# Mathiasb17/Nereus

Hardware: AMD Instinct MI355X
Metric: particle-steps/sec, SESPH dam-break (higher is better)
Workload: dtype f32

## Files before the change

### include/nereus_hip.h

```cpp
#ifndef NEREUS_HIP_H
#define NEREUS_HIP_H

#include <stddef.h>
#include <stdint.h>

#ifdef __cplusplus
extern "C" {
#endif

typedef struct nrs_params_f32 {
    uint32_t gridSize[3];
    uint32_t numCells;
    float worldOrigin[3];
    float cellSize[3];
    uint32_t numBodies;
    uint32_t maxParticlesPerCell;
    float gasStiffness, viscosity, surfaceTension, restDensity, particleMass, interactionRadius, timestep,
        particleRadius;
    float gravity[3];
    float soundSpeed;
    float beta;
    float kpoly, kpoly_grad, kpress_grad, kvisc_grad, kvisc_denum, ksurf1, ksurf2, bpol;
} nrs_params_f32;

// ... 14 lines not shown

typedef struct nrs_ctx nrs_ctx;

enum { NRS_SOLVER_SESPH = 0, NRS_SOLVER_IISPH = 1, NRS_SOLVER_PCISPH = 2, NRS_SOLVER_PBF = 3, NRS_SOLVER_DFSPH = 4 };
enum { NRS_KERNELS_MONAGHAN = 0, NRS_KERNELS_MULLER = 1 };

enum {
    NRS_FLAG_REFERENCE_ORDER = 1u << 0,
    NRS_FLAG_NO_FUSION = 1u << 2,
    NRS_FLAG_NO_SHARED_LISTS = 1u << 3,
    NRS_FLAG_FULL_SORT = 1u << 4,
    NRS_FLAG_FAST_ARITH = 1u << 5,
    NRS_FLAG_IISPH_SELF_BY_SLOT = 1u << 6,
    NRS_FLAG_NO_WALL_WORKGROUPS = 1u << 7,
    NRS_FLAG_STAGED_SCAN = 1u << 8,
    NRS_FLAG_IISPH_INPLACE_P = 1u << 1,
};

enum {
    NRS_OK = 0,
    NRS_E_INVALID = -1,
    NRS_E_HIP = -2,
    NRS_E_CAPACITY = -3,
    NRS_E_STATE = -4,
    NRS_E_NODEVICE = -5,
    NRS_E_NOTREADY = -6,
};

typedef struct nrs_config {
    uint32_t struct_size;
// ... 115 lines not shown

int nrs_slab_configure(nrs_ctx *ctx, int32_t cell_lo, int32_t cell_hi, int32_t halo_cells);
int nrs_slab_pack(nrs_ctx *ctx, void *send_left, void *send_right, uint64_t capacity, uint32_t counts[6]);
int nrs_slab_unpack(nrs_ctx *ctx, const void *recv_left, const void *recv_right, uint64_t capacity);
int nrs_slab_last_counts(nrs_ctx *ctx, uint32_t counts[6]);
uint64_t nrs_num_owned(nrs_ctx *ctx);
uint64_t nrs_slab_message_bytes(uint64_t capacity, int precision);
int nrs_slab_histogram(nrs_ctx *ctx, int32_t first_cell, uint32_t ncells, uint32_t *counts);

int nrs_iisph_predict(nrs_ctx *ctx);
int nrs_iisph_iterate(nrs_ctx *ctx, double *sum_density_corr, uint64_t *count);
int nrs_iisph_finish(nrs_ctx *ctx);

int nrs_resort_stats(nrs_ctx *ctx, uint64_t *steps, uint64_t *fallbacks);

enum { NRS_STAT_MOVERS = 0, NRS_STAT_HIT_OVERFLOW = 1, NRS_STAT_HIT_MEAN = 2, NRS_STAT_HIT_MAX = 3, NRS_STAT_UNSTAGED = 4,
       NRS_STAT_DENSITY_ERROR = 5, NRS_STAT_PCISPH_DELTA = 6, NRS_STAT_PBF_EPSILON = 7, NRS_STAT_DFSPH_DENSITY_AVG = 8,
       NRS_STAT_DFSPH_DIVERGENCE_AVG = 9, NRS_STAT_DFSPH_DIVERGENCE_ITERATIONS = 10, NRS_STAT_SLAB_PARTITION = 11 };
int nrs_get_stat(nrs_ctx *ctx, int which, double *out);

enum { NRS_FIELD_DENSITY = 1, NRS_FIELD_GRADIENT = 2, NRS_FIELD_VELOCITY = 4, NRS_FIELD_COUNT = 8, NRS_FIELD_WALLS = 16 };
typedef struct nrs_lattice { double origin[3]; double spacing[3]; uint32_t dims[3]; uint32_t reserved; } nrs_lattice;
int nrs_sample_points(nrs_ctx *ctx, const void *points4, uint64_t m, uint32_t fields);
int nrs_sample_lattice(nrs_ctx *ctx, const nrs_lattice *lattice, uint32_t fields);
int nrs_sample_result(nrs_ctx *ctx, uint32_t field, void *dst, uint64_t dst_bytes, uint64_t *out_bytes);
int nrs_sample_device_ptr(nrs_ctx *ctx, uint32_t field, void **dptr, uint64_t *bytes);
int nrs_sample_release(nrs_ctx *ctx);
int nrs_sample_builds(nrs_ctx *ctx, uint64_t *builds);

enum { NRS_SURFACE_GRADIENT = 1, NRS_SURFACE_VELOCITY = 2, NRS_SURFACE_WALLS = 4 };
// ... 68 lines not shown
```

### nereus_amd/capi.py

```python
import ctypes as C
import os

import numpy as np

from .params import params_dtype

_HERE = os.path.dirname(os.path.abspath(__file__))
LIB_PATH = os.environ.get("NEREUS_HIP_LIB") or os.path.join(_HERE, "libnereus_hip.so")

SESPH, IISPH, PCISPH, PBF, DFSPH = 0, 1, 2, 3, 4
MONAGHAN, MULLER = 0, 1
FLAG_REFERENCE_ORDER = 1
FLAG_NO_FUSION = 4
FLAG_NO_SHARED_LISTS = 8
FLAG_FULL_SORT = 16
FLAG_FAST_ARITH = 32
FLAG_IISPH_SELF_BY_SLOT = 64
FLAG_NO_WALL_WORKGROUPS = 128
FLAG_STAGED_SCAN = 256
MAX_BODIES = 16
E_NOTREADY = -6
STAT_MOVERS, STAT_HIT_OVERFLOW, STAT_HIT_MEAN, STAT_HIT_MAX, STAT_UNSTAGED = 0, 1, 2, 3, 4
STAT_DENSITY_ERROR, STAT_PCISPH_DELTA, STAT_PBF_EPSILON = 5, 6, 7
STAT_DFSPH_DENSITY_AVG, STAT_DFSPH_DIVERGENCE_AVG, STAT_DFSPH_DIVERGENCE_ITERATIONS = 8, 9, 10
STAT_SLAB_PARTITION = 11
FIELD_DENSITY, FIELD_GRADIENT, FIELD_VELOCITY, FIELD_COUNT, FIELD_WALLS = 1, 2, 4, 8, 16
SURFACE_GRADIENT, SURFACE_VELOCITY, SURFACE_WALLS = 1, 2, 4
MESH_VERTICES, MESH_TRIANGLES, MESH_GRADIENT, MESH_VELOCITY = 1, 2, 4, 8
ANISO_CENTER, ANISO_G, ANISO_COUNT, ANISO_INDEX = 1, 2, 4, 8
DIFFUSE_POS, DIFFUSE_VEL, DIFFUSE_KIND, DIFFUSE_POTENTIALS, DIFFUSE_BIRTHS, DIFFUSE_NORMALS = 0, 1, 2, 3, 4, 5
DIFFUSE_SPRAY, DIFFUSE_FOAM, DIFFUSE_BUBBLE = 0, 1, 2
MAX_EMITTERS, MAX_SINK_BOXES = 16, 16
EMITTER_RECT, EMITTER_DISC = 0, 1
SINK_DOMAIN = 1
# ... 11 lines not shown
    "cellStart": (5, "u"), "cellEnd": (6, "u"), "sortedPos": (7, "v4"), "sortedVel": (8, "v4"),
    "dens": (9, "s"), "pres": (10, "s"), "forces": (11, "v4"), "bhash": (12, "u"), "bindex": (13, "u"),
    "bCellStart": (14, "u"), "bCellEnd": (15, "u"), "bSorted": (16, "v4"),
    "densAdv": (20, "s"), "densCorr": (21, "s"), "P_l": (22, "s"), "aii": (23, "s"), "velAdv": (24, "v4"),
    "forcesAdv": (25, "v4"), "forcesP": (26, "v4"), "diiFluid": (27, "v4"), "diiBoundary": (28, "v4"),
    "sumDij": (29, "v4"), "posPred": (30, "v4"), "vorticity": (31, "v4"), "dfsphAlpha": (32, "s"), "dfsphKappaV": (33, "s"),
    "normals": (34, "v4"), "b_body": (35, "u"),
}

EXPORTS = [
    "nrs_last_error", "nrs_version", "nrs_device_count", "nrs_create", "nrs_destroy", "nrs_set_params",
    "nrs_get_params", "nrs_upload_particles", "nrs_set_num_particles", "nrs_num_particles", "nrs_set_boundaries",
    "nrs_step", "nrs_step_partial", "nrs_synchronize", "nrs_download", "nrs_get_array", "nrs_device_ptr",
    "nrs_last_iterations", "nrs_set_max_iterations", "nrs_set_profiling", "nrs_stage_ms", "nrs_max_density",
    "nrs_max_velocity", "nrs_slab_configure", "nrs_slab_pack", "nrs_slab_unpack", "nrs_num_owned",
    "nrs_slab_message_bytes", "nrs_slab_histogram", "nrs_resort_stats", "nrs_snapshot_begin", "nrs_snapshot_wait",
    "nrs_get_stat", "nrs_boundary_volumes", "nrs_eval_smoothing", "nrs_iisph_predict", "nrs_iisph_iterate", "nrs_iisph_finish",
    "nrs_slab_last_counts", "nrs_pcisph_configure", "nrs_pbf_configure", "nrs_pbf_set_tensile",
    "nrs_pbf_set_vorticity", "nrs_dfsph_configure", "nrs_set_surface_akinci",
    "nrs_set_boundary_bodies", "nrs_set_body_velocity", "nrs_set_body_pose", "nrs_get_body_pose",
    "nrs_sample_points", "nrs_sample_lattice", "nrs_sample_result", "nrs_sample_device_ptr", "nrs_sample_release",
    "nrs_sample_builds",
    "nrs_surface_extract", "nrs_surface_result", "nrs_surface_device_ptr", "nrs_surface_release",
    "nrs_aniso_build", "nrs_aniso_result", "nrs_aniso_device_ptr", "nrs_aniso_release", "nrs_surface_extract_aniso",
    "nrs_diffuse_configure", "nrs_diffuse_step", "nrs_diffuse_count", "nrs_diffuse_result", "nrs_diffuse_device_ptr",
    "nrs_diffuse_upload", "nrs_diffuse_release",
    "nrs_emitter_set", "nrs_emitter_get", "nrs_emit_block", "nrs_sinks_set", "nrs_cull", "nrs_sinks_count",
]


class NrsAnisoConfig(C.Structure):
# ... 88 lines not shown
    lib.nrs_set_surface_akinci.argtypes = [vp, C.c_double, C.c_double]
    lib.nrs_set_profiling.argtypes = [vp, C.c_uint32]
    lib.nrs_stage_ms.argtypes = [vp, i32, C.POINTER(C.c_float), C.POINTER(C.c_uint32)]
    lib.nrs_max_density.argtypes = [vp, C.POINTER(C.c_double)]
    lib.nrs_max_velocity.argtypes = [vp, C.POINTER(C.c_double)]
    lib.nrs_slab_configure.argtypes = [vp, C.c_int32, C.c_int32, C.c_int32]
    lib.nrs_slab_pack.argtypes = [vp, vp, vp, u64, C.POINTER(C.c_uint32)]
    lib.nrs_slab_unpack.argtypes = [vp, vp, vp, u64]
    lib.nrs_slab_last_counts.argtypes = [vp, C.POINTER(C.c_uint32)]
    lib.nrs_num_owned.argtypes = [vp]
    lib.nrs_num_owned.restype = u64
    lib.nrs_slab_message_bytes.argtypes = [u64, i32]
    lib.nrs_slab_message_bytes.restype = u64
    lib.nrs_slab_histogram.argtypes = [vp, C.c_int32, C.c_uint32, C.POINTER(C.c_uint32)]
    lib.nrs_resort_stats.argtypes = [vp, C.POINTER(u64), C.POINTER(u64)]
    lib.nrs_get_stat.argtypes = [vp, i32, C.POINTER(C.c_double)]
    lib.nrs_iisph_predict.argtypes = [vp]
    lib.nrs_iisph_iterate.argtypes = [vp, C.POINTER(C.c_double), C.POINTER(u64)]
    lib.nrs_iisph_finish.argtypes = [vp]
    lib.nrs_eval_smoothing.argtypes = [i32, i32, u64, vp, vp, C.c_double, C.c_double, C.c_double, vp]
    lib.nrs_boundary_volumes.argtypes = [i32, i32, vp, u64, C.c_double, vp]
    lib.nrs_snapshot_begin.argtypes = [vp, i32]
    lib.nrs_snapshot_wait.argtypes = [vp, i32, C.POINTER(vp), C.POINTER(vp), C.POINTER(u64), C.POINTER(u64)]
    lib.nrs_sample_points.argtypes = [vp, vp, u64, C.c_uint32]
    lib.nrs_sample_lattice.argtypes = [vp, C.POINTER(NrsLattice), C.c_uint32]
    lib.nrs_sample_result.argtypes = [vp, C.c_uint32, vp, u64, C.POINTER(u64)]
    lib.nrs_sample_device_ptr.argtypes = [vp, C.c_uint32, C.POINTER(vp), C.POINTER(u64)]
    lib.nrs_sample_release.argtypes = [vp]
    lib.nrs_sample_builds.argtypes = [vp, C.POINTER(u64)]
    lib.nrs_surface_extract.argtypes = [vp, C.POINTER(NrsLattice), C.c_double, C.c_uint32, C.POINTER(u64), C.POINTER(u64)]
# ... 257 lines not shown
        self._chk(rc)
        ct = C.c_double if self.real == np.float64 else C.c_float

        def view(ptr):
            if not ptr.value or not n.value:
                return np.empty((0, 4), self.real) if ptr.value or not n.value else None
            return np.ctypeslib.as_array(C.cast(ptr, C.POINTER(ct)), shape=(int(n.value), 4))

        return view(pp), (view(pv) if pv.value else None), int(step.value)

    def resort_stats(self):
        a, b = C.c_uint64(0), C.c_uint64(0)
        self._chk(self.lib.nrs_resort_stats(self.h, C.byref(a), C.byref(b)))
        return int(a.value), int(b.value)

    def iisph_predict(self):
        self._chk(self.lib.nrs_iisph_predict(self.h))

    def iisph_iterate(self):
        sm, cnt = C.c_double(0), C.c_uint64(0)
        self._chk(self.lib.nrs_iisph_iterate(self.h, C.byref(sm), C.byref(cnt)))
        return sm.value, int(cnt.value)

    def iisph_finish(self):
        self._chk(self.lib.nrs_iisph_finish(self.h))

    def get_stat(self, which):
        v = C.c_double()
        self._chk(self.lib.nrs_get_stat(self.h, int(which), C.byref(v)))
        return v.value
# ... 209 lines not shown
```

### nereus_amd/csrc/nrs_abi.hip

```cpp
#include "nrs_ctx_base.h"

#include <condition_variable>
#include <mutex>
#include <thread>

namespace nrs {

thread_local std::string g_err;

enum { KS_MONAGHAN_ = 0, KS_MULLER_ = 1 };
extern template CtxBase *make_ctx2<float, KS_MULLER_>(bool);
extern template CtxBase *make_ctx2<float, KS_MONAGHAN_>(bool);
extern template CtxBase *make_ctx2<double, KS_MULLER_>(bool);
extern template CtxBase *make_ctx2<double, KS_MONAGHAN_>(bool);

static CtxBase *make_ctx(const nrs_config &c)
{
    if (c.precision == 32) return c.kernel_set == NRS_KERNELS_MULLER ? make_ctx2<float, KS_MULLER_>(c.surface_tension != 0) : make_ctx2<float, KS_MONAGHAN_>(c.surface_tension != 0);
    return c.kernel_set == NRS_KERNELS_MULLER ? make_ctx2<double, KS_MULLER_>(c.surface_tension != 0) : make_ctx2<double, KS_MONAGHAN_>(c.surface_tension != 0);
}

}

using namespace nrs;
// ... 343 lines not shown
    ctx->wait_idle();
    ctx->settle_keep_error();
    return ctx->impl->num_owned();
}
int nrs_slab_histogram(nrs_ctx *ctx, int32_t first_cell, uint32_t ncells, uint32_t *counts)
{
    CTX_GUARD(ctx);
    return ctx->impl->slab_histogram(first_cell, ncells, counts);
}
int nrs_resort_stats(nrs_ctx *ctx, uint64_t *steps, uint64_t *fallbacks)
{
    CTX_GUARD(ctx);
    ctx->impl->resort_stats(steps, fallbacks);
    return NRS_OK;
}
int nrs_iisph_predict(nrs_ctx *ctx)
{
    CTX_GUARD(ctx);
    return ctx->impl->iisph_phase(0, nullptr, nullptr);
}
int nrs_iisph_iterate(nrs_ctx *ctx, double *sum_density_corr, uint64_t *count)
{
    CTX_GUARD(ctx);
    return ctx->impl->iisph_phase(1, sum_density_corr, count);
}
int nrs_iisph_finish(nrs_ctx *ctx)
{
    CTX_GUARD(ctx);
    return ctx->impl->iisph_phase(2, nullptr, nullptr);
}
// ... 170 lines not shown
```

### nereus_amd/csrc/nrs_ctx_base.h

```cpp
#pragma once
#include <cstring>
#include <hip/hip_runtime.h>

#include <cmath>
#include <cstdio>
#include <string>
#include <type_traits>
#include <utility>
#include <vector>

#include "nrs_error.h"

namespace nrs {

#define HIPCHK(expr)                                                                                     \
    do {                                                                                                 \
        hipError_t e_ = (expr);                                                                          \
        if (e_ != hipSuccess)                                                                            \
            return fail(NRS_E_HIP, std::string(#expr) + ": " + hipGetErrorString(e_) + " (" __FILE__ ":" + \
                                       std::to_string(__LINE__) + ")");                                  \
    } while (0)

struct DevBuf {
    void *p = nullptr;
// ... 75 lines not shown
    virtual int get_body_pose(uint32_t body, double *x, double *q) = 0;
    virtual int step(int nsteps, int stop) = 0;
    virtual int sync() = 0;
    virtual int download(void *pos4, void *vel4, void *pres) = 0;
    virtual int snapshot_begin(int withVel) = 0;
    virtual int snapshot_wait(int block, const void **pos4, const void **vel4, uint64_t *n, uint64_t *step) = 0;
    virtual int array(int which, void **dptr, uint64_t *bytes) = 0;
    virtual int stage_ms(int stage, float *ms, uint32_t *launches) = 0;
    virtual int reduce_max(int which, double *out) = 0;
    virtual int slab_configure(int lo, int hi, int halo) = 0;
    virtual int slab_pack(void *sendL, void *sendR, uint64_t cap, uint32_t *counts) = 0;
    virtual int slab_unpack(const void *recvL, const void *recvR, uint64_t cap) = 0;
    virtual uint64_t num_owned() = 0;
    virtual int slab_histogram(int lo0, uint32_t nbins, uint32_t *out) = 0;
    virtual void resort_stats(uint64_t *steps, uint64_t *fallbacks) = 0;
    virtual int get_stat(int which, double *out) = 0;
    virtual int iisph_phase(int phase, double *sum, uint64_t *count) = 0;
    virtual int pcisph_configure(double eta, uint32_t minIters, double spacing, double delta) = 0;
    virtual int pbf_configure(double eta, uint32_t minIters, double relaxation, double xsph) = 0;
    virtual int pbf_set_tensile(double k, double dq) = 0;
    virtual int pbf_set_vorticity(double epsV) = 0;
    virtual int dfsph_configure(double eta, uint32_t minIters, double etaV, uint32_t minItersV, int warm) = 0;
    virtual int set_surface_akinci(double gamma, double beta) = 0;
    virtual int settle() = 0;
    virtual int slab_last_counts(uint32_t *counts) = 0;
    virtual int set_profiling(uint32_t mask) = 0;
    virtual int sample_points(const void *points4, uint64_t m, uint32_t fields) = 0;
    virtual int sample_lattice(const nrs_lattice *lattice, uint32_t fields) = 0;
    virtual int sample_result(uint32_t field, void *dst, uint64_t dstBytes, uint64_t *outBytes) = 0;
    virtual int sample_device_ptr(uint32_t field, void **dptr, uint64_t *bytes) = 0;
// ... 36 lines not shown
```

### nereus_amd/csrc/nrs_ctx_impl.h

```cpp
#pragma once
#include "nrs_ctx_base.h"
#include "nrs_boundary_tables.h"
#include "nrs_host_grid.h"
#include "nrs_host_plan.h"
#include "nrs_host_profile.h"
#include "nrs_host_settings.h"
#include "nrs_host_slab.h"
#include "nrs_host_snapshot.h"
#include "nrs_host_solver.h"
#include "nrs_host_state.h"
#include "nrs_sort.h"
#include "nrs_wall_list.h"

#include "nrs_kernels_ref.h"
#include "nrs_kernels_tiled.h"
#include "nrs_kernels_staged.h"
#include <type_traits>
#include "nrs_kernels_iisph.h"
#include "nrs_kernels_pcisph.h"
#include "nrs_kernels_pbf.h"
#include "nrs_kernels_dfsph.h"
#include "nrs_kernels_akinci.h"
#include "nrs_kernels_bodies.h"
#include "nrs_slab_exchange.h"
// ... 22 lines not shown
        qOk = P.gridSize[0] >= 4u;
        for (int a = 0; a < 3; ++a) {
            qc.o[a] = (double)P.worldOrigin[a];
            qc.s[a] = QP_PER_CELL / (float)P.cellSize[a];
            const float r = (float)P.interactionRadius * qc.s[a];
            qOk = qOk && P.cellSize[a] > (R)0 && std::isfinite(qc.s[a]) && (r + QP_MARGIN < QP_HALF);
            hq = std::max(hq, r);
        }
        const double lim = (double)hq + (double)QP_MARGIN;
        qT = qOk ? (uint32_t)std::ceil(lim * lim) + 1u : 0u;
    }
    QuantCfg qc;
    uint32_t qT = 0;
    bool qOk = false;
    DevBuf gatherPos;
    DevBuf qpos;
    nrs_config cfg;
    uint64_t cap = 0, n = 0;
    bool midStep = false;
    DevBuf posA, posB, velA, velB, presA, presB, dens, forces;
    DevBuf inv;
    SortStage sort;
    DevBuf cellStart, cellEnd;
    uint32_t cellsAllocated = 0;
    BoundaryTables<R> bt;
    DevBuf densAdv, densCorr, P_l, P_l2, aii, velAdv, forcesAdv, forcesP, diiF, diiB, sumDij, diiSum;
    DevBuf redPartial, redOut;
    DevBuf posPred, posPred2, pciErr;
    DevBuf dfAlpha, dfKvA, dfKvB, dfErrV;
    DevBuf pbfVort, akNormals;
// ... 387 lines not shown
        splitClearedCells = clear;
        st.split_queued();
        NRSCHK(ev_end());
        return NRS_OK;
    }

    template <bool HAS_B> int sesph_tail(int stop)
    {
        const uint32_t N = (uint32_t)n;
        const dim3 g(nblocks(N)), b(BLOCK);
        GridView<R> G = grid_view();
        if (exch.on()) { G.actLo = exch.cuts().lo - 1; G.actHi = exch.cuts().hi + 1; }
        HitBuffer hb = hit_buffer();
        hb.gpos = gatherPos.p; hb.gvel = gatherPos.as<T4>() + 1; hb.svel = velB.p;
        if (plan.fast && !plan.staged) hb.fast = fastQ.as<FastPair>();
        const HitBuffer *share = plan.lists ? &hb : nullptr;
        const WallList wv = wall_view();
        const WallList *walls = plan.walls ? &wv : nullptr;
        if (plan.walls) {
            NRSCHK(ev_begin(NRS_STAGE_REORDER, true));
            NRSCHK(build_wall_list(N));
            NRSCHK(ev_end());
        }
        NRSCHK(ev_begin(NRS_STAGE_DENSITY));
        if (plan.ref) {
            hipLaunchKernelGGL((k_density_ref<R, KSET, HAS_B>), g, b, 0, stream, P, G, posB.as<T4>(), dens.as<R>(), presB.as<R>(), N);
        } else if (plan.staged) {
            if constexpr (std::is_same<R, float>::value)
                launch_density_staged<KSET, HAS_B>(stream, P, G, share, plan.fast, posB.as<T4>(), dens.as<R>(), presB.as<R>(),
                                                   plan.fast ? fastQ.as<FastPair>() : (FastPair *)nullptr, N);
// ... 25 lines not shown
                st.classified(N);
                sort.tile_counts_written();
            }
        }
        const FusedOut<R> *fused = plan.keys ? &fo : nullptr;
        T4 *out = plan.keys ? (T4 *)nullptr : forces.as<T4>();
        if (plan.ref) {
            hipLaunchKernelGGL((k_forces_ref<R, KSET, SURF, HAS_B>), g, b, 0, stream, P, G, posB.as<T4>(), velB.as<T4>(),
                               dens.as<R>(), presB.as<R>(), out, N);
        } else if (plan.fast) {
            if constexpr (std::is_same<R, float>::value && KSET == KS_MULLER)
                launch_forces_fast<SURF, HAS_B>(stream, P, G, hb, posB.as<T4>(), velB.as<T4>(), dens.as<R>(), presB.as<R>(),
                                                fastQ.as<FastPair>(), out, fused, N);
        } else {
            launch_forces_tiled<R, KSET, SURF, HAS_B>(stream, P, G, share, posB.as<T4>(), velB.as<T4>(), dens.as<R>(), presB.as<R>(), out,
                                                      fused, N, walls);
        }
        if (plan.keys) {
            if (!exch.on()) keys_ready();
            else sort.keys_written();
            fusedThisStep = true;
        }
        NRSCHK(ev_end());
        if (plan.resort) NRSCHK(queue_resort_split(N));
        if (stop == NRS_STAGE_FORCES || plan.keys) return NRS_OK;
        NRSCHK(ev_begin(NRS_STAGE_INTEGRATE));
        hipLaunchKernelGGL((k_integrate<R>), g, b, 0, stream, P, posB.as<T4>(), velB.as<T4>(), forces.as<T4>(), N);
        NRSCHK(ev_end());
        return NRS_OK;
    }

// ... 684 lines not shown
        st.arrivals_appended(ar.inplace, (uint32_t)ar.arrivals);
        if (!ar.inplace && st.fields().hashReady && compactResort && n >= RESORT_MIN_PARTICLES) {
            const uint32_t N = (uint32_t)n;
            NRSCHK(sort.scan_movers(nblocks(N), false));
            NRSCHK(sort.split(SplitFrom::PACKED, N, nullptr));
            st.split_queued_known(exch.host().totals[ST_CHANGED] + ar.start[5]);
        }
        exch.unpack_done();
        return NRS_OK;
    }

    void resort_stats(uint64_t *steps, uint64_t *fallbacks) override
    {
        if (steps) *steps = sort.stats().steps;
        if (fallbacks) *fallbacks = sort.stats().fallbacks;
    }
    StatFacts stat_facts() const
    {
        return StatFacts{cfg.solver, exch.host().packed, pbfSt.errPending != 0, !(pciSt.lastErr < 0.0), dfSt.denN, dfSt.divN, hitCounts.p != nullptr, n != 0, midStep};
    }
    int get_stat(int which, double *out) override
    {
        StatRoute r;
        NRSCHK(route_stat(which, stat_facts(), r));
        if (r.formMaxFirst) {
            NRSCHK(max_of<false>(pciErr.p, pbfSt.errPending, &pciSt.lastErr));
            pbfSt.errPending = 0;
            NRSCHK(route_stat(which, stat_facts(), r));
        }
        switch (r.kind) {
// ... 310 lines not shown
```

### nereus_amd/csrc/nrs_host_plan.h

```cpp
#pragma once
#include <cstdint>

#include "nrs_error.h"
#include "nrs_host_state.h"

namespace nrs {

struct PlanFacts {
    uint32_t flags;
    int solver;
    bool muller;
    bool fp32;
    uint64_t cap, n;
    bool qOk;
    bool pow2Grid;
    bool nearBitsValid;
    bool walls;
    bool slabOn;
    uint32_t numCells;
};
struct Features {
    bool listKernels;
    bool lists;
    bool fast;
// ... 6 lines not shown
    Features ft;
    ft.listKernels = sesph || a.muller;
    ft.lists = ft.listKernels && !(f & (NRS_FLAG_REFERENCE_ORDER | NRS_FLAG_NO_SHARED_LISTS));
    ft.fast = ft.lists && (f & NRS_FLAG_FAST_ARITH) && sesph && a.fp32 && a.muller;
    ft.resort = !(f & (NRS_FLAG_REFERENCE_ORDER | NRS_FLAG_NO_FUSION | NRS_FLAG_FULL_SORT)) && a.cap >= RESORT_MIN_PARTICLES;
    return ft;
}
struct StepPlan {
    bool ref = true;
    bool quant = false;
    bool lists = false;
    bool wallTiles = false;
    bool walls = false;
    bool staged = false;
    bool fast = false;
    bool keys = false;
    bool resort = false;
    bool classify = false;
    bool watch = false;
};
static inline StepPlan plan_step(const PlanFacts &a, int stop, bool ref)
{
    const Features ft = plan_features(a);
    const bool sesph = a.solver == NRS_SOLVER_SESPH, iisph = a.solver == NRS_SOLVER_IISPH;
    StepPlan s;
    s.ref = ref || (a.flags & NRS_FLAG_REFERENCE_ORDER) || !a.pow2Grid;
    s.quant = ft.lists && a.qOk;
    if (s.ref) return s;
    s.lists = s.quant && (!sesph || stop != NRS_STAGE_DENSITY);
    s.staged = (a.flags & NRS_FLAG_STAGED_SCAN) && a.fp32 && a.muller && sesph && s.quant && a.numCells <= (1u << 30);
    s.fast = ft.fast && s.lists;
    s.wallTiles = !(a.flags & NRS_FLAG_NO_WALL_WORKGROUPS) && a.nearBitsValid && a.walls && s.quant && !s.staged;
    s.walls = s.wallTiles && s.lists;
    s.keys = stop == 0 && !(a.flags & NRS_FLAG_NO_FUSION) && !(iisph && a.slabOn);
    const bool resort = s.keys && ft.resort && a.n >= RESORT_MIN_PARTICLES;
    s.resort = resort && !a.slabOn;
    s.classify = resort && a.slabOn;
    s.watch = iisph && s.lists && !a.slabOn;
    return s;
}

template <typename Iterate, typename Measure>
int solve_loop(bool fixed, uint32_t minIters, uint32_t cap, double eta, Iterate &&iterate, Measure &&measure, uint32_t *iters, double *err)
{
    uint32_t l = 0;
    for (;;) {
// ... 16 lines not shown
```

### nereus_amd/csrc/nrs_kernels_tiled.h

```cpp
#pragma once
#include "nrs_kernels_ref.h"
#include "nrs_kernels_slab.h"
#include <type_traits>

namespace nrs {

constexpr int HIT_CAP = 20;
constexpr uint32_t HIT_INDEX = (1u << 27) - 1;
constexpr int HIT_TAG_SHIFT = 27;

struct CutThresholds { float lenLtIr, r2LeH2; };

#ifndef FORCES_LISTS_MIN_WAVES
#define FORCES_LISTS_MIN_WAVES 7
#endif
#ifndef FORCES_PACKED_MIN_WAVES
#define FORCES_PACKED_MIN_WAVES 5
#endif
#ifndef FORCES_PACKED_MIN_WAVES_UNFUSED
#define FORCES_PACKED_MIN_WAVES_UNFUSED 4
#endif
NRS_DEV float bcast_lane(float v, int srcLane) { return __int_as_float(__builtin_amdgcn_readlane(__float_as_int(v), srcLane)); }
NRS_DEV double bcast_lane(double v, int srcLane)
{
// ... 13 lines not shown
#ifndef QP_PRE
#define QP_PRE 2
#endif
constexpr int SCAN_CAP = 21;
NRS_DEV int mad24(int a, int b, int c)
{
    int d;
    asm("v_mad_i32_i24 %0, %1, %2, %3" : "=v"(d) : "v"(a), "v"(b), "v"(c));
    return d;
}
constexpr int SCAN_BATCH = 4;

struct HitCounts { int nf, nb; bool over; bool anyB; };
constexpr uint32_t GATHER_STRIDE = 2u;
template <typename R> struct PrePair { R prq, mrho; };

template <typename R> struct Sweep {
    typedef typename Vec4T<R>::type T4;
    static NRS_DEV T4 at32(const T4 *__restrict__ base, uint32_t idx)
    {
        const uint32_t off = idx * (uint32_t)sizeof(T4);
        return *reinterpret_cast<const T4 *>(reinterpret_cast<const char *>(base) + off);
    }

    template <bool HAS_B, int BFILT, int W, bool FWIDE = false>
    static NRS_DEV HitCounts scan(const Params<R> &P, const GridView<R> &G, const CutThresholds thr,
                                  const T4 *__restrict__ sPos, uint32_t self, V3<R> p, uint32_t (*lst)[W])
    {
        const I3 gp = calcGridPos<R>(P, p);
        const uint32_t mx = P.gridSize[0] - 1, my = P.gridSize[1] - 1, mz = P.gridSize[2] - 1;
// ... 461 lines not shown
NRS_DEV void walk_fluid_batched(const uint32_t *col, uint32_t stride, int nf, GATHER &&gather, USE &&use)
{
    for (int k0 = 0; k0 < nf; k0 += NB) {
        uint32_t e[NB];
        decltype(gather(0u)) d[NB];
#pragma unroll
        for (int u = 0; u < NB; ++u) e[u] = col[(size_t)min(k0 + u, nf - 1) * stride];
#pragma unroll
        for (int u = 0; u < NB; ++u) d[u] = gather(e[u] & HIT_INDEX);
#pragma unroll
        for (int u = 0; u < NB; ++u)
            if (k0 + u < nf) use(e[u] & HIT_INDEX, e[u] >> HIT_TAG_SHIFT, d[u]);
    }
}

template <typename R, int KSET, bool SURF, bool HAS_B, bool STRICT = false, bool PAIRS = false, bool BOUNDARY_BY_CELL = false>
NRS_DEV ForceAcc<R> forces_from_hits(const Params<R> &P, const GridView<R> &G,
                                     const typename Vec4T<R>::type *__restrict__ sPos,
                                     const typename Vec4T<R>::type *__restrict__ sVel, const R *__restrict__ sDens,
                                     const R *__restrict__ sPres, V3<R> pos1, V3<R> vel1, R dens, R pres,
                                     const uint32_t *lbase, uint32_t lstride, HitCounts hc, uint32_t self = 0xffffffffu,
                                     const R *pre = nullptr, const typename Vec4T<R>::type *__restrict__ gpos = nullptr,
                                     const typename Vec4T<R>::type *__restrict__ gvel = nullptr, const uint32_t *__restrict__ lroot = nullptr,
                                     uint32_t lcol = 0u)
{
    ForceAcc<R> A;
    A.fpres = A.fvisc = A.fsurf = A.fbound = mk3<R>(0, 0, 0);
    const R pm = P.particleMass, m2 = P.particleMass, ir = P.interactionRadius, kp = P.kpoly;
    const R kappa = P.surfaceTension;
    const R kprg = P.kpress_grad, kvg = P.kvisc_grad, kvd = P.kvisc_denum;
    const R diameter = (R)(2.0 * P.particleRadius);
    const R diameter2 = diameter * diameter;
    const R rhoSqOwn = dens * dens;
    R wAtDiameter;
    if (KSET == KS_MONAGHAN) wAtDiameter = Wmonaghan<R>(mk3<R>(diameter, 0, 0), ir);
    else wAtDiameter = Wdefault<R>(mk3<R>(diameter, 0, 0), ir, kp);
    const R epsilon = (R)0.01;
    const R beta = P.beta, rd = P.restDensity;
    auto boundaryHit = [&](const BoundaryTerms<R, KSET> &T) {
// ... 67 lines not shown
        return A;
    }
    if constexpr (!HAS_B && !STRICT && PAIRS && KSET == KS_MULLER && std::is_same<R, float>::value) {
        const int nf = hc.nf;
        const float own = pres / rhoSqOwn, c0 = kappa / pm * pm;
        auto walk = [&](auto inRange, const InRange &IG, bool &bad) {
            ForceAcc<R> S;
            S.fpres = S.fvisc = S.fsurf = S.fbound = mk3<R>(0, 0, 0);
            auto entry = [&](int k) { return lroot[(size_t)k * lstride + lcol]; };
            uint32_t e0 = nf > 0 ? entry(0) : 0u, e1 = nf > 1 ? entry(1) : e0;
            for (int k = 0; k < nf; k += 2) {
                const uint32_t j0 = e0 & HIT_INDEX, j1 = e1 & HIT_INDEX;
                const bool two = k + 1 < nf;
                const uint32_t n0 = k + 2 < nf ? entry(k + 2) : 0u;
                const uint32_t n1 = k + 3 < nf ? entry(k + 3) : n0;
                const float4 pa = gpos[GATHER_STRIDE * j0], pb = gpos[GATHER_STRIDE * j1], va = gvel[GATHER_STRIDE * j0], vb = gvel[GATHER_STRIDE * j1];
                const PairTerms2 T = fluid_terms2_muller<SURF, decltype(inRange)::value>(P, pos1, vel1, own, c0, wAtDiameter, diameter2, pa, pb, va, vb,
                                                                                        PrePair<float>{pa.w, va.w}, PrePair<float>{pb.w, vb.w}, IG, bad);
                S.fpres = S.fpres + mk3<R>(T.pres.x.x, T.pres.y.x, T.pres.z.x);
                S.fvisc = S.fvisc + mk3<R>(T.visc.x.x, T.visc.y.x, T.visc.z.x);
                if (SURF) S.fsurf = S.fsurf + mk3<R>(T.surf.x.x, T.surf.y.x, T.surf.z.x);
                if (two) {
                    S.fpres = S.fpres + mk3<R>(T.pres.x.y, T.pres.y.y, T.pres.z.y);
                    S.fvisc = S.fvisc + mk3<R>(T.visc.x.y, T.visc.y.y, T.visc.z.y);
                    if (SURF) S.fsurf = S.fsurf + mk3<R>(T.surf.x.y, T.surf.y.y, T.surf.z.y);
                }
                e0 = n0; e1 = n1;
            }
            return S;
        };
        const InRange IG = in_range_setup(P);
// ... 79 lines not shown
        over += __shfl_down(over, d);
        sum += __shfl_down(sum, d);
        unst += __shfl_down(unst, d);
        const unsigned long long o = __shfl_down(mx, d);
        mx = o > mx ? o : mx;
    }
    if ((threadIdx.x & 63u) == 0) {
        atomicAdd(&out[0], over);
        atomicAdd(&out[1], sum);
        atomicMax(&out[2], mx);
        atomicAdd(&out[3], unst);
    }
}

constexpr uint32_t COUNTS_DEFERRED = 1u << 19;

NRS_DEV bool cell_near_boundary(const WallList &wl, uint32_t h) { return ((wl.nearBits[h >> 5] >> (h & 31u)) & 1u) != 0u; }

static __global__ __launch_bounds__(BLOCK) void k_wall_compact(WallList wl, const uint32_t *__restrict__ tileOffset, const uint32_t *__restrict__ groupPrefix,
                                                                 uint32_t groupSize, uint32_t *__restrict__ list, uint32_t n)
{
    __shared__ uint32_t waveCnt[BLOCK / 64];
    const uint32_t i = blockIdx.x * BLOCK + threadIdx.x, lane = threadIdx.x & 63u, wave = threadIdx.x >> 6;
    const unsigned long long m = wl.mask[i >> 6];
    const bool take = ((m >> lane) & 1ull) != 0ull;
    if (lane == 0) waveCnt[wave] = (uint32_t)__popcll(m);
    __syncthreads();
    if (!take) return;
    uint32_t before = (uint32_t)__popcll(m & ((1ull << lane) - 1ull));
    for (uint32_t w = 0; w < wave; ++w) before += waveCnt[w];
// ... 155 lines not shown
    const T4 v4 = sVel[i];
    const V3<R> pos1 = xyz<R>(p4), vel1 = xyz<R>(v4);
    V3<R> f = mk3<R>(0, 0, 0);
    if (slab_active<R>(P, G, pos1.x)) {
        const R dens = sDens[i], pres = sPres[i];
        constexpr int BF = (KSET == KS_MULLER ? 1 : 2);
        const HitCounts hc = Sweep<R>::template scan<HAS_B, BF, BLOCK>(P, G, thr, sPos, i, pos1, lst);
        ForceAcc<R> A;
        if (hc.over) A = gather_forces<R, KSET, SURF, HAS_B>(P, G, i, pos1, vel1, dens, pres, sPos, sVel, sDens, sPres);
        else A = forces_from_hits<R, KSET, SURF, HAS_B, false, false, (HAS_B && BF == 2)>(P, G, sPos, sVel, sDens, sPres, pos1, vel1, dens, pres, &lst[0][tid], BLOCK, hc);
        f = sesph_total_force<R>(P, A, dens);
    }
    forces_epilogue<R, KSET, SURF, HAS_B, FUSE>(P, p4, v4, f, forces, fo, i);
}

template <typename R, int KSET, bool SURF, bool HAS_B, bool FUSE>
NRS_DEV void forces_lists_particle(const Params<R> &P, const GridView<R> &G, const HitBuffer &hb,
                                   const typename Vec4T<R>::type *__restrict__ sPos, const typename Vec4T<R>::type *__restrict__ sVel,
                                   const R *__restrict__ sDens, const R *__restrict__ sPres, typename Vec4T<R>::type *__restrict__ forces,
                                   const FusedOut<R> &fo, uint32_t i, typename Vec4T<R>::type p4, typename Vec4T<R>::type v4,
                                   bool active, HitCounts hc)
{
    const V3<R> pos1 = xyz<R>(p4), vel1 = xyz<R>(v4);
    V3<R> f = mk3<R>(0, 0, 0);
    if (active) {
        const R dens = sDens[i], pres = sPres[i];
        ForceAcc<R> A;
        if (hc.over) A = gather_forces<R, KSET, SURF, HAS_B>(P, G, i, pos1, vel1, dens, pres, sPos, sVel, sDens, sPres);
        else
            A = forces_from_hits<R, KSET, SURF, HAS_B, false, true, (HAS_B && KSET == KS_MONAGHAN)>(P, G, sPos, sVel, sDens, sPres, pos1, vel1, dens, pres, hb.hits + i, hb.stride,
                                                                                     hc, 0xffffffffu, nullptr, reinterpret_cast<const typename Vec4T<R>::type *>(hb.gpos),
                                                                                     reinterpret_cast<const typename Vec4T<R>::type *>(hb.gvel), hb.hits, i);
        f = sesph_total_force<R>(P, A, dens);
    }
    forces_epilogue<R, KSET, SURF, HAS_B, FUSE>(P, p4, v4, f, forces, fo, i);
}

template <typename R, int KSET, bool SURF, bool HAS_B, bool FUSE, bool DEFER = false>
__global__ __launch_bounds__(BLOCK, (sizeof(R) == 4 ? ((KSET == KS_MULLER && !HAS_B) ? (FUSE ? FORCES_PACKED_MIN_WAVES : FORCES_PACKED_MIN_WAVES_UNFUSED) : FORCES_LISTS_MIN_WAVES) : 1)) void k_forces_lists(Params<R> P, GridView<R> G, HitBuffer hb,
                                                        const typename Vec4T<R>::type *__restrict__ sPos,
                                                        const typename Vec4T<R>::type *__restrict__ sVel,
                                                        const R *__restrict__ sDens, const R *__restrict__ sPres,
                                                        typename Vec4T<R>::type *__restrict__ forces, FusedOut<R> fo,
                                                        uint32_t n, WallList wl, uint32_t wallBlocks)
{
    typedef typename Vec4T<R>::type T4;
    uint32_t block = blockIdx.x, blocks = gridDim.x;
    if (DEFER) {
        if (block < wallBlocks) {
            const uint32_t count = *wl.count;
            for (uint32_t t = block * BLOCK + threadIdx.x; t < count; t += wallBlocks * BLOCK) {
                const uint32_t i = wl.list[t];
                const T4 p4 = sPos[i];
                const bool active = slab_active<R>(P, G, p4.x);
                forces_lists_particle<R, KSET, SURF, true, FUSE>(P, G, hb, sPos, sVel, sDens, sPres, forces, fo, i, p4, sVel[i], active,
                                                                 unpack_counts(active ? hb.counts[i] : 0u));
            }
            return;
        }
        block -= wallBlocks; blocks -= wallBlocks;
    }
    const uint32_t i = xcd_tile(block, blocks) * BLOCK + threadIdx.x;
    if (i >= n) return;
    const uint32_t c = hb.counts[i];
    if (DEFER && (c & COUNTS_DEFERRED)) return;
    const T4 p4 = sPos[i];
    const bool active = slab_active<R>(P, G, p4.x);
    forces_lists_particle<R, KSET, SURF, HAS_B, FUSE>(P, G, hb, sPos, sVel, sDens, sPres, forces, fo, i, p4, sVel[i], active,
                                                      unpack_counts(active ? c : 0u));
}

template <typename R>
__global__ __launch_bounds__(BLOCK) void k_mark_near_boundary(Params<R> P, const uint32_t *__restrict__ bHash, uint32_t nb, uint32_t *__restrict__ nearBits)
{
    const uint32_t i = blockIdx.x * BLOCK + threadIdx.x;
    if (i >= nb) return;
    const uint32_t h = bHash[i];
// ... 61 lines not shown
    const CutThresholds thr = make_thresholds<R>(P);
    const uint32_t g = (n + BLOCK - 1) / BLOCK;
    if (HAS_B && wall) {
        const uint32_t wb = wall_blocks(g);
        hipLaunchKernelGGL((k_density_tiled<R, KSET, false, true, true, true>), dim3(g + wb), dim3(BLOCK), 0, stream, P, G, thr, sPos, dens,
                           (R *)nullptr, hb, n, *wall, wb);
        return;
    }
    hipLaunchKernelGGL((k_density_tiled<R, KSET, HAS_B, true, true>), dim3(g), dim3(BLOCK), 0, stream, P, G, thr,
                       sPos, dens, (R *)nullptr, hb, n, WallList{}, 0u);
}
template <typename R, int KSET, bool SURF, bool HAS_B>
static inline void launch_forces_tiled(hipStream_t stream, const Params<R> &P, const GridView<R> &G, const HitBuffer *lists,
                                       const typename Vec4T<R>::type *sPos, const typename Vec4T<R>::type *sVel, const R *dens,
                                       const R *pres, typename Vec4T<R>::type *forces, const FusedOut<R> *fused, uint32_t n,
                                       const WallList *wall = nullptr)
{
    const FusedOut<R> fo = fused ? *fused : FusedOut<R>{};
    const dim3 g((n + BLOCK - 1) / BLOCK), b(BLOCK);
    constexpr unsigned padF = NRS_DBG_LDS_PAD_F;
    if (lists && HAS_B && wall) {
        const uint32_t wb = wall_blocks(g.x);
        const dim3 gd(g.x + wb);
        if (fused) hipLaunchKernelGGL((k_forces_lists<R, KSET, SURF, false, true, true>), gd, b, padF, stream, P, G, *lists, sPos, sVel, dens, pres, forces, fo, n, *wall, wb);
        else hipLaunchKernelGGL((k_forces_lists<R, KSET, SURF, false, false, true>), gd, b, 0, stream, P, G, *lists, sPos, sVel, dens, pres, forces, fo, n, *wall, wb);
    } else if (lists) {
        if (fused) hipLaunchKernelGGL((k_forces_lists<R, KSET, SURF, HAS_B, true>), g, b, padF, stream, P, G, *lists, sPos, sVel, dens, pres, forces, fo, n, WallList{}, 0u);
        else hipLaunchKernelGGL((k_forces_lists<R, KSET, SURF, HAS_B, false>), g, b, 0, stream, P, G, *lists, sPos, sVel, dens, pres, forces, fo, n, WallList{}, 0u);
    } else {
        const CutThresholds thr = make_thresholds<R>(P);
        if (fused) hipLaunchKernelGGL((k_forces_tiled<R, KSET, SURF, HAS_B, true>), g, b, 0, stream, P, G, thr, sPos, sVel, dens, pres, forces, fo, n);
        else hipLaunchKernelGGL((k_forces_tiled<R, KSET, SURF, HAS_B, false>), g, b, 0, stream, P, G, thr, sPos, sVel, dens, pres, forces, fo, n);
    }
}

// ... 2 lines not shown
```

Baseline: 5.016 billion.

## Stage per-wave neighbour window in LDS for SESPH force list walk

Each wavefront of the packed list-based force kernel loads a contiguous window of gathered position/velocity records, its own 64 particles plus a 16-particle margin on each side, into LDS. Neighbour fetches that fall inside the window read from LDS, and the rest fall back to global gathers. This aims to cut scattered global-memory traffic, since sorted neighbours are often index-close. It costs LDS per wave, a preload and wave barrier, and a branch per fetch. The change also adds a diagnostic counter API and a flag to disable the window.

New measurement: 5.109 billion, median of 6. +1.9%, better.

```diff
diff --git a/include/nereus_hip.h b/include/nereus_hip.h
--- a/include/nereus_hip.h
+++ b/include/nereus_hip.h
@@ -52,6 +52,7 @@
     NRS_FLAG_IISPH_SELF_BY_SLOT = 1u << 6,
     NRS_FLAG_NO_WALL_WORKGROUPS = 1u << 7,
     NRS_FLAG_STAGED_SCAN = 1u << 8,
+    NRS_FLAG_NO_FORCE_WINDOW = 1u << 9,
     NRS_FLAG_IISPH_INPLACE_P = 1u << 1,
 };
 
@@ -197,6 +198,8 @@
 
 int nrs_resort_stats(nrs_ctx *ctx, uint64_t *steps, uint64_t *fallbacks);
 
+int nrs_force_window_counts(nrs_ctx *ctx, uint64_t out[3]);
+
 enum { NRS_STAT_MOVERS = 0, NRS_STAT_HIT_OVERFLOW = 1, NRS_STAT_HIT_MEAN = 2, NRS_STAT_HIT_MAX = 3, NRS_STAT_UNSTAGED = 4,
        NRS_STAT_DENSITY_ERROR = 5, NRS_STAT_PCISPH_DELTA = 6, NRS_STAT_PBF_EPSILON = 7, NRS_STAT_DFSPH_DENSITY_AVG = 8,
        NRS_STAT_DFSPH_DIVERGENCE_AVG = 9, NRS_STAT_DFSPH_DIVERGENCE_ITERATIONS = 10, NRS_STAT_SLAB_PARTITION = 11 };
diff --git a/nereus_amd/capi.py b/nereus_amd/capi.py
--- a/nereus_amd/capi.py
+++ b/nereus_amd/capi.py
@@ -18,6 +18,7 @@
 FLAG_IISPH_SELF_BY_SLOT = 64
 FLAG_NO_WALL_WORKGROUPS = 128
 FLAG_STAGED_SCAN = 256
+FLAG_NO_FORCE_WINDOW = 512
 MAX_BODIES = 16
 E_NOTREADY = -6
 STAT_MOVERS, STAT_HIT_OVERFLOW, STAT_HIT_MEAN, STAT_HIT_MAX, STAT_UNSTAGED = 0, 1, 2, 3, 4
@@ -59,7 +60,7 @@
     "nrs_step", "nrs_step_partial", "nrs_synchronize", "nrs_download", "nrs_get_array", "nrs_device_ptr",
     "nrs_last_iterations", "nrs_set_max_iterations", "nrs_set_profiling", "nrs_stage_ms", "nrs_max_density",
     "nrs_max_velocity", "nrs_slab_configure", "nrs_slab_pack", "nrs_slab_unpack", "nrs_num_owned",
-    "nrs_slab_message_bytes", "nrs_slab_histogram", "nrs_resort_stats", "nrs_snapshot_begin", "nrs_snapshot_wait",
+    "nrs_slab_message_bytes", "nrs_slab_histogram", "nrs_resort_stats", "nrs_force_window_counts", "nrs_snapshot_begin", "nrs_snapshot_wait",
     "nrs_get_stat", "nrs_boundary_volumes", "nrs_eval_smoothing", "nrs_iisph_predict", "nrs_iisph_iterate", "nrs_iisph_finish",
     "nrs_slab_last_counts", "nrs_pcisph_configure", "nrs_pbf_configure", "nrs_pbf_set_tensile",
     "nrs_pbf_set_vorticity", "nrs_dfsph_configure", "nrs_set_surface_akinci",
@@ -178,6 +179,7 @@
     lib.nrs_slab_message_bytes.restype = u64
     lib.nrs_slab_histogram.argtypes = [vp, C.c_int32, C.c_uint32, C.POINTER(C.c_uint32)]
     lib.nrs_resort_stats.argtypes = [vp, C.POINTER(u64), C.POINTER(u64)]
+    lib.nrs_force_window_counts.argtypes = [vp, C.POINTER(u64)]
     lib.nrs_get_stat.argtypes = [vp, i32, C.POINTER(C.c_double)]
     lib.nrs_iisph_predict.argtypes = [vp]
     lib.nrs_iisph_iterate.argtypes = [vp, C.POINTER(C.c_double), C.POINTER(u64)]
@@ -465,6 +467,11 @@
         self._chk(self.lib.nrs_resort_stats(self.h, C.byref(a), C.byref(b)))
         return int(a.value), int(b.value)
 
+    def force_window_counts(self):
+        out = (C.c_uint64 * 3)()
+        self._chk(self.lib.nrs_force_window_counts(self.h, out))
+        return int(out[0]), int(out[1]), int(out[2])
+
     def iisph_predict(self):
         self._chk(self.lib.nrs_iisph_predict(self.h))
 
diff --git a/nereus_amd/csrc/nrs_abi.hip b/nereus_amd/csrc/nrs_abi.hip
--- a/nereus_amd/csrc/nrs_abi.hip
+++ b/nereus_amd/csrc/nrs_abi.hip
@@ -381,6 +381,12 @@
     ctx->impl->resort_stats(steps, fallbacks);
     return NRS_OK;
 }
+int nrs_force_window_counts(nrs_ctx *ctx, uint64_t out[3])
+{
+    CTX_GUARD(ctx);
+    if (!out) return fail(NRS_E_INVALID, "out is null");
+    return ctx->impl->force_window_counts(out);
+}
 int nrs_iisph_predict(nrs_ctx *ctx)
 {
     CTX_GUARD(ctx);
diff --git a/nereus_amd/csrc/nrs_ctx_base.h b/nereus_amd/csrc/nrs_ctx_base.h
--- a/nereus_amd/csrc/nrs_ctx_base.h
+++ b/nereus_amd/csrc/nrs_ctx_base.h
@@ -113,6 +113,7 @@
     virtual uint64_t num_owned() = 0;
     virtual int slab_histogram(int lo0, uint32_t nbins, uint32_t *out) = 0;
     virtual void resort_stats(uint64_t *steps, uint64_t *fallbacks) = 0;
+    virtual int force_window_counts(uint64_t out[3]) = 0;
     virtual int get_stat(int which, double *out) = 0;
     virtual int iisph_phase(int phase, double *sum, uint64_t *count) = 0;
     virtual int pcisph_configure(double eta, uint32_t minIters, double spacing, double delta) = 0;
diff --git a/nereus_amd/csrc/nrs_ctx_impl.h b/nereus_amd/csrc/nrs_ctx_impl.h
--- a/nereus_amd/csrc/nrs_ctx_impl.h
+++ b/nereus_amd/csrc/nrs_ctx_impl.h
@@ -60,6 +60,8 @@
     uint32_t qT = 0;
     bool qOk = false;
     DevBuf gatherPos;
+    bool windowRan = false;
+    uint64_t windowN = 0, windowGen = 0;
     DevBuf qpos;
     nrs_config cfg;
     uint64_t cap = 0, n = 0;
@@ -477,6 +479,8 @@
         HitBuffer hb = hit_buffer();
         hb.gpos = gatherPos.p; hb.gvel = gatherPos.as<T4>() + 1; hb.svel = velB.p;
         if (plan.fast && !plan.staged) hb.fast = fastQ.as<FastPair>();
+        const bool window = plan.window && (!HAS_B || plan.walls);
+        windowRan = false;
         const HitBuffer *share = plan.lists ? &hb : nullptr;
         const WallList wv = wall_view();
         const WallList *walls = plan.walls ? &wv : nullptr;
@@ -532,7 +536,8 @@
                                                 fastQ.as<FastPair>(), out, fused, N);
         } else {
             launch_forces_tiled<R, KSET, SURF, HAS_B>(stream, P, G, share, posB.as<T4>(), velB.as<T4>(), dens.as<R>(), presB.as<R>(), out,
-                                                      fused, N, walls);
+                                                      fused, N, walls, window);
+            if (window) { windowRan = true; windowN = N; windowGen = particleGen; }
         }
         if (plan.keys) {
             if (!exch.on()) keys_ready();
@@ -1247,6 +1252,20 @@
     {
         if (steps) *steps = sort.stats().steps;
         if (fallbacks) *fallbacks = sort.stats().fallbacks;
+    }
+    int force_window_counts(uint64_t out[3]) override
+    {
+        if (!windowRan || windowN != n || windowGen != particleGen)
+            return fail(NRS_E_STATE, "the last step ran without the force walk's LDS window");
+        const HitBuffer hb = hit_buffer();
+        const uint32_t N = (uint32_t)n;
+        HIPCHK(hipMemsetAsync(redPartial.p, 0, 3 * sizeof(unsigned long long), stream));
+        hipLaunchKernelGGL(k_force_window_counts, dim3(std::min<uint32_t>(1024u, nblocks(N))), dim3(BLOCK), 0, stream, hb, (unsigned long long *)redPartial.p, N);
+        unsigned long long h[3] = {0, 0, 0};
+        HIPCHK(hipMemcpyAsync(h, redPartial.p, sizeof(h), hipMemcpyDeviceToHost, stream));
+        HIPCHK(hipStreamSynchronize(stream));
+        for (int k = 0; k < 3; ++k) out[k] = h[k];
+        return NRS_OK;
     }
     StatFacts stat_facts() const
     {
diff --git a/nereus_amd/csrc/nrs_host_plan.h b/nereus_amd/csrc/nrs_host_plan.h
--- a/nereus_amd/csrc/nrs_host_plan.h
+++ b/nereus_amd/csrc/nrs_host_plan.h
@@ -44,6 +44,7 @@
     bool walls = false;
     bool staged = false;
     bool fast = false;
+    bool window = false;
     bool keys = false;
     bool resort = false;
     bool classify = false;
@@ -60,6 +61,7 @@
     s.lists = s.quant && (!sesph || stop != NRS_STAGE_DENSITY);
     s.staged = (a.flags & NRS_FLAG_STAGED_SCAN) && a.fp32 && a.muller && sesph && s.quant && a.numCells <= (1u << 30);
     s.fast = ft.fast && s.lists;
+    s.window = s.lists && !s.fast && !s.staged && sesph && a.fp32 && a.muller && !(a.flags & NRS_FLAG_NO_FORCE_WINDOW);
     s.wallTiles = !(a.flags & NRS_FLAG_NO_WALL_WORKGROUPS) && a.nearBitsValid && a.walls && s.quant && !s.staged;
     s.walls = s.wallTiles && s.lists;
     s.keys = stop == 0 && !(a.flags & NRS_FLAG_NO_FUSION) && !(iisph && a.slabOn);
diff --git a/nereus_amd/csrc/nrs_kernels_tiled.h b/nereus_amd/csrc/nrs_kernels_tiled.h
--- a/nereus_amd/csrc/nrs_kernels_tiled.h
+++ b/nereus_amd/csrc/nrs_kernels_tiled.h
@@ -51,6 +51,18 @@
 struct HitCounts { int nf, nb; bool over; bool anyB; };
 constexpr uint32_t GATHER_STRIDE = 2u;
 template <typename R> struct PrePair { R prq, mrho; };
+
+constexpr uint32_t WINDOW_MARGIN = 16u;
+constexpr uint32_t WINDOW_POOL = 64u + 2u * WINDOW_MARGIN;
+struct ForceWindow { uint32_t L, len; };
+NRS_DEV uint32_t uniform_u32(uint32_t v) { return (uint32_t)__builtin_amdgcn_readfirstlane((int)v); }
+NRS_DEV ForceWindow force_window_of(uint32_t wave, uint32_t n)
+{
+    ForceWindow W;
+    W.L = max(wave * 64u, WINDOW_MARGIN) - WINDOW_MARGIN;
+    W.len = min(wave * 64u + 64u + WINDOW_MARGIN, n) - W.L;
+    return W;
+}
 
 template <typename R> struct Sweep {
     typedef typename Vec4T<R>::type T4;
@@ -542,7 +554,7 @@
     }
 }
 
-template <typename R, int KSET, bool SURF, bool HAS_B, bool STRICT = false, bool PAIRS = false, bool BOUNDARY_BY_CELL = false>
+template <typename R, int KSET, bool SURF, bool HAS_B, bool STRICT = false, bool PAIRS = false, bool BOUNDARY_BY_CELL = false, bool WINDOW = false>
 NRS_DEV ForceAcc<R> forces_from_hits(const Params<R> &P, const GridView<R> &G,
                                      const typename Vec4T<R>::type *__restrict__ sPos,
                                      const typename Vec4T<R>::type *__restrict__ sVel, const R *__restrict__ sDens,
@@ -550,7 +562,7 @@
                                      const uint32_t *lbase, uint32_t lstride, HitCounts hc, uint32_t self = 0xffffffffu,
                                      const R *pre = nullptr, const typename Vec4T<R>::type *__restrict__ gpos = nullptr,
                                      const typename Vec4T<R>::type *__restrict__ gvel = nullptr, const uint32_t *__restrict__ lroot = nullptr,
-                                     uint32_t lcol = 0u)
+                                     uint32_t lcol = 0u, ForceWindow win = ForceWindow{}, const float4 *pool = nullptr)
 {
     ForceAcc<R> A;
     A.fpres = A.fvisc = A.fsurf = A.fbound = mk3<R>(0, 0, 0);
@@ -648,7 +660,21 @@
                 const bool two = k + 1 < nf;
                 const uint32_t n0 = k + 2 < nf ? entry(k + 2) : 0u;
                 const uint32_t n1 = k + 3 < nf ? entry(k + 3) : n0;
-                const float4 pa = gpos[GATHER_STRIDE * j0], pb = gpos[GATHER_STRIDE * j1], va = gvel[GATHER_STRIDE * j0], vb = gvel[GATHER_STRIDE * j1];
+                float4 pa, pb, va, vb;
+                if constexpr (WINDOW) {
+                    auto fetch = [&](uint32_t j, float4 &p, float4 &v) {
+                        const uint32_t d = j - win.L;
+                        if (d < win.len) {
+                            p = pool[GATHER_STRIDE * d]; v = pool[GATHER_STRIDE * d + 1u];
+                        } else {
+                            p = gpos[GATHER_STRIDE * j]; v = gvel[GATHER_STRIDE * j];
+                        }
+                    };
+                    fetch(j0, pa, va);
+                    fetch(j1, pb, vb);
+                } else {
+                    pa = gpos[GATHER_STRIDE * j0]; pb = gpos[GATHER_STRIDE * j1]; va = gvel[GATHER_STRIDE * j0]; vb = gvel[GATHER_STRIDE * j1];
+                }
                 const PairTerms2 T = fluid_terms2_muller<SURF, decltype(inRange)::value>(P, pos1, vel1, own, c0, wAtDiameter, diameter2, pa, pb, va, vb,
                                                                                         PrePair<float>{pa.w, va.w}, PrePair<float>{pb.w, vb.w}, IG, bad);
                 S.fpres = S.fpres + mk3<R>(T.pres.x.x, T.pres.y.x, T.pres.z.x);
@@ -758,6 +784,33 @@
 }
 
 constexpr uint32_t COUNTS_DEFERRED = 1u << 19;
+
+static __global__ __launch_bounds__(BLOCK) void k_force_window_counts(HitBuffer hb, unsigned long long *__restrict__ out, uint32_t n)
+{
+    unsigned long long all = 0, central = 0, staged = 0;
+    for (uint32_t i = blockIdx.x * BLOCK + threadIdx.x; i < n; i += gridDim.x * BLOCK) {
+        const ForceWindow W = force_window_of(i >> 6, n);
+        const uint32_t c = hb.counts[i];
+        const HitCounts hc = unpack_counts(c);
+        if ((c & COUNTS_DEFERRED) || hc.over) continue;
+        for (int k = 0; k < hc.nf; ++k) {
+            const uint32_t e = hb.hits[(size_t)k * hb.stride + i], j = e & HIT_INDEX, tag = e >> HIT_TAG_SHIFT;
+            ++all;
+            central += (tag >= 9u && tag <= 17u) ? 1ull : 0ull;
+            staged += (j - W.L < W.len) ? 1ull : 0ull;
+        }
+    }
+    for (int d = 32; d >= 1; d >>= 1) {
+        all += __shfl_down(all, d);
+        central += __shfl_down(central, d);
+        staged += __shfl_down(staged, d);
+    }
+    if ((threadIdx.x & 63u) == 0) {
+        atomicAdd(&out[0], all);
+        atomicAdd(&out[1], central);
+        atomicAdd(&out[2], staged);
+    }
+}
 
 NRS_DEV bool cell_near_boundary(const WallList &wl, uint32_t h) { return ((wl.nearBits[h >> 5] >> (h & 31u)) & 1u) != 0u; }
 
@@ -943,12 +996,12 @@
     forces_epilogue<R, KSET, SURF, HAS_B, FUSE>(P, p4, v4, f, forces, fo, i);
 }
 
-template <typename R, int KSET, bool SURF, bool HAS_B, bool FUSE>
+template <typename R, int KSET, bool SURF, bool HAS_B, bool FUSE, bool WINDOW = false>
 NRS_DEV void forces_lists_particle(const Params<R> &P, const GridView<R> &G, const HitBuffer &hb,
                                    const typename Vec4T<R>::type *__restrict__ sPos, const typename Vec4T<R>::type *__restrict__ sVel,
                                    const R *__restrict__ sDens, const R *__restrict__ sPres, typename Vec4T<R>::type *__restrict__ forces,
                                    const FusedOut<R> &fo, uint32_t i, typename Vec4T<R>::type p4, typename Vec4T<R>::type v4,
-                                   bool active, HitCounts hc)
+                                   bool active, HitCounts hc, ForceWindow win = ForceWindow{}, const float4 *pool = nullptr)
 {
     const V3<R> pos1 = xyz<R>(p4), vel1 = xyz<R>(v4);
     V3<R> f = mk3<R>(0, 0, 0);
@@ -957,15 +1010,15 @@
         ForceAcc<R> A;
         if (hc.over) A = gather_forces<R, KSET, SURF, HAS_B>(P, G, i, pos1, vel1, dens, pres, sPos, sVel, sDens, sPres);
         else
-            A = forces_from_hits<R, KSET, SURF, HAS_B, false, true, (HAS_B && KSET == KS_MONAGHAN)>(P, G, sPos, sVel, sDens, sPres, pos1, vel1, dens, pres, hb.hits + i, hb.stride,
+            A = forces_from_hits<R, KSET, SURF, HAS_B, false, true, (HAS_B && KSET == KS_MONAGHAN), WINDOW>(P, G, sPos, sVel, sDens, sPres, pos1, vel1, dens, pres, hb.hits + i, hb.stride,
                                                                                      hc, 0xffffffffu, nullptr, reinterpret_cast<const typename Vec4T<R>::type *>(hb.gpos),
-                                                                                     reinterpret_cast<const typename Vec4T<R>::type *>(hb.gvel), hb.hits, i);
+                                                                                     reinterpret_cast<const typename Vec4T<R>::type *>(hb.gvel), hb.hits, i, win, pool);
         f = sesph_total_force<R>(P, A, dens);
     }
     forces_epilogue<R, KSET, SURF, HAS_B, FUSE>(P, p4, v4, f, forces, fo, i);
 }
 
-template <typename R, int KSET, bool SURF, bool HAS_B, bool FUSE, bool DEFER = false>
+template <typename R, int KSET, bool SURF, bool HAS_B, bool FUSE, bool DEFER = false, bool WINDOW = false>
 __global__ __launch_bounds__(BLOCK, (sizeof(R) == 4 ? ((KSET == KS_MULLER && !HAS_B) ? (FUSE ? FORCES_PACKED_MIN_WAVES : FORCES_PACKED_MIN_WAVES_UNFUSED) : FORCES_LISTS_MIN_WAVES) : 1)) void k_forces_lists(Params<R> P, GridView<R> G, HitBuffer hb,
                                                         const typename Vec4T<R>::type *__restrict__ sPos,
                                                         const typename Vec4T<R>::type *__restrict__ sVel,
@@ -990,6 +1043,36 @@
         block -= wallBlocks; blocks -= wallBlocks;
     }
     const uint32_t i = xcd_tile(block, blocks) * BLOCK + threadIdx.x;
+    if constexpr (WINDOW) {
+        static_assert(std::is_same<R, float>::value && KSET == KS_MULLER && !HAS_B, "the window serves the packed walk");
+        __shared__ float4 pools[BLOCK / 64][GATHER_STRIDE * WINDOW_POOL];
+        float4 *const pool = pools[uniform_u32(threadIdx.x >> 6)];
+        const uint32_t wave = uniform_u32(i >> 6);
+        if (wave * 64u >= n) return;
+        const ForceWindow W = force_window_of(wave, n);
+        const float4 *__restrict__ rec = reinterpret_cast<const float4 *>(hb.gpos) + (size_t)GATHER_STRIDE * W.L;
+        const uint32_t last = GATHER_STRIDE * W.len - 1u;
+        uint32_t t[3];
+        float4 v[3];
+#pragma unroll
+        for (int u = 0; u < 3; ++u) {
+            t[u] = min((threadIdx.x & 63u) + 64u * (uint32_t)u, last);
+            v[u] = rec[t[u]];
+        }
+#pragma unroll
+        for (int u = 0; u < 3; ++u) pool[t[u]] = v[u];
+        __builtin_amdgcn_fence(__ATOMIC_RELEASE, "wavefront");
+        __builtin_amdgcn_wave_barrier();
+        __builtin_amdgcn_fence(__ATOMIC_ACQUIRE, "wavefront");
+        if (i >= n) return;
+        const uint32_t c = hb.counts[i];
+        if (DEFER && (c & COUNTS_DEFERRED)) return;
+        const T4 p4 = sPos[i];
+        const bool active = slab_active<R>(P, G, p4.x);
+        forces_lists_particle<R, KSET, SURF, HAS_B, FUSE, true>(P, G, hb, sPos, sVel, sDens, sPres, forces, fo, i, p4, sVel[i], active,
+                                                                unpack_counts(active ? c : 0u), W, pool);
+        return;
+    }
     if (i >= n) return;
     const uint32_t c = hb.counts[i];
     if (DEFER && (c & COUNTS_DEFERRED)) return;
@@ -1081,11 +1164,25 @@
 static inline void launch_forces_tiled(hipStream_t stream, const Params<R> &P, const GridView<R> &G, const HitBuffer *lists,
                                        const typename Vec4T<R>::type *sPos, const typename Vec4T<R>::type *sVel, const R *dens,
                                        const R *pres, typename Vec4T<R>::type *forces, const FusedOut<R> *fused, uint32_t n,
-                                       const WallList *wall = nullptr)
+                                       const WallList *wall = nullptr, bool window = false)
 {
     const FusedOut<R> fo = fused ? *fused : FusedOut<R>{};
     const dim3 g((n + BLOCK - 1) / BLOCK), b(BLOCK);
     constexpr unsigned padF = NRS_DBG_LDS_PAD_F;
+    if constexpr (std::is_same<R, float>::value && KSET == KS_MULLER) {
+        if (window && lists && HAS_B && wall) {
+            const uint32_t wb = wall_blocks(g.x);
+            const dim3 gd(g.x + wb);
+            if (fused) hipLaunchKernelGGL((k_forces_lists<R, KSET, SURF, false, true, true, true>), gd, b, padF, stream, P, G, *lists, sPos, sVel, dens, pres, forces, fo, n, *wall, wb);
+            else hipLaunchKernelGGL((k_forces_lists<R, KSET, SURF, false, false, true, true>), gd, b, 0, stream, P, G, *lists, sPos, sVel, dens, pres, forces, fo, n, *wall, wb);
+            return;
+        }
+        if (window && lists && !HAS_B) {
+            if (fused) hipLaunchKernelGGL((k_forces_lists<R, KSET, SURF, false, true, false, true>), g, b, padF, stream, P, G, *lists, sPos, sVel, dens, pres, forces, fo, n, WallList{}, 0u);
+            else hipLaunchKernelGGL((k_forces_lists<R, KSET, SURF, false, false, false, true>), g, b, 0, stream, P, G, *lists, sPos, sVel, dens, pres, forces, fo, n, WallList{}, 0u);
+            return;
+        }
+    }
     if (lists && HAS_B && wall) {
         const uint32_t wb = wall_blocks(g.x);
         const dim3 gd(g.x + wb);
```
